# tensorchord/VectorChord-bm25

Hardware: AMD Instinct MI355X
Metric: queries/sec top-10 BM25, 10M synthetic docs; achieved HBM GB/s vs peak (higher is better)
Workload: dtype f64

## Files before the change

vectorchord-bm25_amd/csrc/scan_win.h:

```cpp
#ifndef VBM25_SCAN_WIN_H
#define VBM25_SCAN_WIN_H

#include "device_types.h"
#include "decode.h"
#include "topk_lds.h"
#include "block_fetch.h"
#include "topk_reg.h"

namespace vbm25 {

#pragma clang diagnostic push
#pragma clang diagnostic ignored "-Winline-asm"
constexpr int WN_T = 8;
#ifndef VBM25_WIN_WAVES_MAX
#define VBM25_WIN_WAVES_MAX 12
#endif
constexpr int wn_wave_lds(int mt) { return 8192 + 512 * mt + 256; }
constexpr int WN_WG_LDS = 2048 + 16;
constexpr int wn_waves(int mt, int rk) {
    const int by_lds = (163840 - WN_WG_LDS) / wn_wave_lds(mt);
    const int by_regs = rk <= 2 && mt <= 3 ? 16 : 12;
    const int n = by_lds < by_regs ? by_lds : by_regs;
    return n < VBM25_WIN_WAVES_MAX ? n : VBM25_WIN_WAVES_MAX;
}
constexpr bool wn_lane_addr(int mt, int rk) { return !(rk == 4 && mt >= 7); }
constexpr int WN_BM_WORDS = 2048;
constexpr int WN_SLOT = 256;
constexpr int WN_LIST = 64;
constexpr uint32_t WN_GRID = 256;

typedef __attribute__((address_space(3))) uint32_t wn_lds_u32;
struct WnBm {
    uint32_t base, mask;
};
__device__ __forceinline__ uint32_t wn_or_rtn(const WnBm bm, const uint32_t x, const uint32_t bit) {
    return __hip_atomic_fetch_or((wn_lds_u32 *)(((x >> 3) & bm.mask) | bm.base), bit, __ATOMIC_RELAXED, __HIP_MEMORY_SCOPE_WORKGROUP);
}
__device__ __forceinline__ void wn_or(const WnBm bm, const uint32_t x, const uint32_t bit) {
    (void)__hip_atomic_fetch_or((wn_lds_u32 *)(((x >> 3) & bm.mask) | bm.base), bit, __ATOMIC_RELAXED, __HIP_MEMORY_SCOPE_WORKGROUP);
}
template <int MT>
struct WinWave {
    alignas(16) uint16_t stage[MT * WN_SLOT];
    uint32_t list[WN_LIST];
};

__device__ __forceinline__ uint32_t wn_mbcnt(unsigned long long mask) {
    return __builtin_amdgcn_mbcnt_hi((uint32_t)(mask >> 32), __builtin_amdgcn_mbcnt_lo((uint32_t)mask, 0u));
}

template <bool RET, int MT>
__device__ __forceinline__ void wn_pair(WinWave<MT> &S, const WnBm bmbase, const uint2 v, const uint32_t r0, const uint32_t n,
                                        const uint32_t t, uint32_t &nd) {
    const uint32_t x0 = v.x & 0xffffu, x1 = v.x >> 16, x2 = v.y & 0xffffu, x3 = v.y >> 16;
    const uint32_t b0 = r0 < n ? 1u << (x0 & 31u) : 0u;
    const uint32_t b1 = r0 + 1u < n ? 1u << (x1 & 31u) : 0u;
    const uint32_t b2 = r0 + 2u < n ? 1u << (x2 & 31u) : 0u;
    const uint32_t b3 = r0 + 3u < n ? 1u << (x3 & 31u) : 0u;
    if (!RET) {
        wn_or(bmbase, x0, b0);
        wn_or(bmbase, x1, b1);
        wn_or(bmbase, x2, b2);
        wn_or(bmbase, x3, b3);
        return;
    }
    const uint32_t h0 = wn_or_rtn(bmbase, x0, b0) & b0;
    const uint32_t h1 = wn_or_rtn(bmbase, x1, b1) & b1;
    const uint32_t h2 = wn_or_rtn(bmbase, x2, b2) & b2;
    const uint32_t h3 = wn_or_rtn(bmbase, x3, b3) & b3;
    if (__ballot((h0 | h1 | h2 | h3) != 0u)) {
        uint32_t hm = (h0 ? 1u : 0u) | (h1 ? 2u : 0u) | (h2 ? 4u : 0u) | (h3 ? 8u : 0u);
        do {
            const bool has = hm != 0u;
            const uint32_t j = (uint32_t)__ffs((int)hm) - 1u;
            hm &= hm - 1u;
            const uint32_t x = j == 0u ? x0 : j == 1u ? x1 : j == 2u ? x2 : x3;
            const unsigned long long mk = __ballot(has);
            const uint32_t pos = nd + wn_mbcnt(mk);
            if (has && pos < (uint32_t)WN_LIST) S.list[pos] = x | t << 16 | 0x80000000u;
            nd += (uint32_t)__popcll(mk);
        } while (__ballot(hm != 0u));
    }
}

__device__ __forceinline__ void wn_load_run(unsigned long long &dst, const uint32_t voff, const unsigned long long sbase) {
    asm volatile("s_nop 4\n\tglobal_load_dwordx2 %0, %1, %2" : "=v"(dst) : "v"(voff), "s"(sbase));
}
__device__ __forceinline__ void wn_load_run_at(unsigned long long &dst, const unsigned long long vaddr) {
    asm volatile("global_load_dwordx2 %0, %1, off" : "=v"(dst) : "v"(vaddr));
}
__device__ __forceinline__ void wn_load_word(uint32_t &dst, const uint32_t *addr) {
    asm volatile("global_load_dword %0, %1, off" : "=v"(dst) : "v"(addr));
}
__device__ __forceinline__ void wn_load_theta(unsigned long long &dst, const uint32_t vzero, const unsigned long long *sbase) {
    asm volatile("s_nop 4\n\tglobal_load_dwordx2 %0, %1, %2 sc1" : "=v"(dst) : "v"(vzero), "s"(sbase));
}
#define WN_STR2(x) #x
#define WN_STR(x) WN_STR2(x)
#define WN_OPS1(b) "+v"(b[0])
#define WN_OPS2(b) WN_OPS1(b), "+v"(b[1])
#define WN_OPS3(b) WN_OPS2(b), "+v"(b[2])
#define WN_OPS4(b) WN_OPS3(b), "+v"(b[3])
#define WN_OPS5(b) WN_OPS4(b), "+v"(b[4])
#define WN_OPS6(b) WN_OPS5(b), "+v"(b[5])
#define WN_OPS7(b) WN_OPS6(b), "+v"(b[6])
#define WN_OPS8(b) WN_OPS7(b), "+v"(b[7])
template <int MT>
__device__ __forceinline__ void wn_wait_runs(unsigned long long (&b)[MT]) {
    static_assert(MT >= 1 && MT <= 8, "operand lists");
    if constexpr (MT == 1) asm volatile("s_waitcnt vmcnt(4)" : WN_OPS1(b));
    if constexpr (MT == 2) asm volatile("s_waitcnt vmcnt(5)" : WN_OPS2(b));
    if constexpr (MT == 3) asm volatile("s_waitcnt vmcnt(6)" : WN_OPS3(b));
    if constexpr (MT == 4) asm volatile("s_waitcnt vmcnt(7)" : WN_OPS4(b));
    if constexpr (MT == 5) asm volatile("s_waitcnt vmcnt(8)" : WN_OPS5(b));
    if constexpr (MT == 6) asm volatile("s_waitcnt vmcnt(9)" : WN_OPS6(b));
    if constexpr (MT == 7) asm volatile("s_waitcnt vmcnt(10)" : WN_OPS7(b));
    if constexpr (MT == 8) asm volatile("s_waitcnt vmcnt(11)" : WN_OPS8(b));
}
template <int MT>
__device__ __forceinline__ void wn_wait_words(uint32_t &ga, uint32_t &gb) {
    if constexpr (MT == 1) asm volatile("s_waitcnt vmcnt(1)" : "+v"(ga), "+v"(gb));
    if constexpr (MT == 2) asm volatile("s_waitcnt vmcnt(2)" : "+v"(ga), "+v"(gb));
    if constexpr (MT == 3) asm volatile("s_waitcnt vmcnt(3)" : "+v"(ga), "+v"(gb));
    if constexpr (MT == 4) asm volatile("s_waitcnt vmcnt(4)" : "+v"(ga), "+v"(gb));
    if constexpr (MT == 5) asm volatile("s_waitcnt vmcnt(5)" : "+v"(ga), "+v"(gb));
    if constexpr (MT == 6) asm volatile("s_waitcnt vmcnt(6)" : "+v"(ga), "+v"(gb));
    if constexpr (MT == 7) asm volatile("s_waitcnt vmcnt(7)" : "+v"(ga), "+v"(gb));
    if constexpr (MT == 8) asm volatile("s_waitcnt vmcnt(8)" : "+v"(ga), "+v"(gb));
}
template <int MT>
__device__ __forceinline__ void wn_wait_theta(unsigned long long &p) {
    if constexpr (MT == 1) asm volatile("s_waitcnt vmcnt(3)" : "+v"(p));
    if constexpr (MT == 2) asm volatile("s_waitcnt vmcnt(4)" : "+v"(p));
    if constexpr (MT == 3) asm volatile("s_waitcnt vmcnt(5)" : "+v"(p));
    if constexpr (MT == 4) asm volatile("s_waitcnt vmcnt(6)" : "+v"(p));
    if constexpr (MT == 5) asm volatile("s_waitcnt vmcnt(7)" : "+v"(p));
    if constexpr (MT == 6) asm volatile("s_waitcnt vmcnt(8)" : "+v"(p));
    if constexpr (MT == 7) asm volatile("s_waitcnt vmcnt(9)" : "+v"(p));
    if constexpr (MT == 8) asm volatile("s_waitcnt vmcnt(10)" : "+v"(p));
}
__device__ __forceinline__ void wn_wait_all(uint32_t &g) { asm volatile("s_waitcnt vmcnt(0)" : "+v"(g)); }
__device__ __forceinline__ unsigned long long wn_load_run_now(const uint16_t *addr) {
    unsigned long long v;
    asm volatile("global_load_dwordx2 %0, %1, off\n\ts_waitcnt vmcnt(0)" : "=v"(v) : "v"(addr));
    return v;
}
__device__ __forceinline__ uint32_t wn_load_u16_now(const uint16_t *addr) {
    uint32_t v;
    asm volatile("global_load_ushort %0, %1, off\n\ts_waitcnt vmcnt(0)" : "=v"(v) : "v"(addr));
    return v;
}
template <int MT>
__device__ __forceinline__ void wn_drain(unsigned long long (&a)[MT], unsigned long long (&b)[MT], uint32_t &g, uint32_t &g2, unsigned long long &p) {
    if constexpr (MT == 1) asm volatile("s_waitcnt vmcnt(0)" : WN_OPS1(a), WN_OPS1(b), "+v"(g), "+v"(g2), "+v"(p));
    if constexpr (MT == 2) asm volatile("s_waitcnt vmcnt(0)" : WN_OPS2(a), WN_OPS2(b), "+v"(g), "+v"(g2), "+v"(p));
    if constexpr (MT == 3) asm volatile("s_waitcnt vmcnt(0)" : WN_OPS3(a), WN_OPS3(b), "+v"(g), "+v"(g2), "+v"(p));
    if constexpr (MT == 4) asm volatile("s_waitcnt vmcnt(0)" : WN_OPS4(a), WN_OPS4(b), "+v"(g), "+v"(g2), "+v"(p));
    if constexpr (MT == 5) asm volatile("s_waitcnt vmcnt(0)" : WN_OPS5(a), WN_OPS5(b), "+v"(g), "+v"(g2), "+v"(p));
    if constexpr (MT == 6) asm volatile("s_waitcnt vmcnt(0)" : WN_OPS6(a), WN_OPS6(b), "+v"(g), "+v"(g2), "+v"(p));
    if constexpr (MT == 7) asm volatile("s_waitcnt vmcnt(0)" : WN_OPS7(a), WN_OPS7(b), "+v"(g), "+v"(g2), "+v"(p));
    if constexpr (MT == 8) asm volatile("s_waitcnt vmcnt(0)" : WN_OPS8(a), WN_OPS8(b), "+v"(g), "+v"(g2), "+v"(p));
}
__device__ __forceinline__ double wave_shl1_f64(double v) {
    const uint32_t lo = (uint32_t)__builtin_amdgcn_update_dpp(__double2loint(v), __double2loint(v), 0x130, 0xf, 0xf, false);
    const uint32_t hi = (uint32_t)__builtin_amdgcn_update_dpp(__double2hiint(v), __double2hiint(v), 0x130, 0xf, 0xf, false);
    return __hiloint2double((int)hi, (int)lo);
}
struct WnPend {
    bool valid, found, task;
    uint32_t x, p, w, gw;
    uint32_t cw;
};

constexpr uint32_t WN_LQ_SCORE = 1024;
constexpr uint32_t WN_LQ_DOC = 1536;
constexpr uint32_t WN_LQ_CNT = 1792;
constexpr uint32_t WN_LQ_G = 3, WN_LQ_WAVES = 12, WN_LQ_STRIDE = 4;
static_assert(WN_LQ_G * 256 <= WN_LQ_SCORE && WN_LQ_CNT + 4 <= 2048, "map, lists and counts share a filter");

template <int RK, bool LQ>
__device__ __forceinline__ void wn_merge_query(const DevIndex &ix, const uint32_t q, const uint32_t g, const uint32_t k, const uint32_t lane,
                                            uint32_t *map, double *sv_score, uint32_t *sv_doc, const uint32_t *lq) {
    const KernArgsP ca = cold_args();
    RegTopK<RK> rtop;
    rtop.init();
    const uint32_t L0 = q * g;
    constexpr uint32_t LQS = WN_LQ_STRIDE * (uint32_t)WN_BM_WORDS;
    unsigned long long theta = 0;
    if constexpr (LQ) {
        for (uint32_t i = 0; i < g; ++i) {
            const unsigned long long ti = (unsigned long long)lq[i * LQS + WN_LQ_CNT + 3u] << 32 | lq[i * LQS + WN_LQ_CNT + 2u];
            if (ti > theta) theta = ti;
        }
    } else {
        theta = __hip_atomic_load(&ca->bt.theta[q], __ATOMIC_RELAXED, __HIP_MEMORY_SCOPE_AGENT);
    }
    const uint32_t per_round = k <= 128u ? 16u : 2048u / k;
    uint32_t nsv = 0;
    bool ranked = true;
    for (uint32_t lb = 0; lb < g; lb += per_round) {
        uint32_t cnt = 0;
        if (lane < per_round && lb + lane < g) {
            if constexpr (LQ) cnt = min(lq[(lb + lane) * LQS + WN_LQ_CNT], k);
            else cnt = min(__hip_atomic_load(&ca->bt.res_cnt[L0 + lb + lane], __ATOMIC_RELAXED, __HIP_MEMORY_SCOPE_AGENT), k);
        }
        const uint32_t incl = wave_incl_scan_u32(cnt), excl = incl - cnt;
        const uint32_t total = (uint32_t)__builtin_amdgcn_readlane((int)incl, 63);
        for (uint32_t j = 0; j < cnt; ++j) map[excl + j] = lane << 16 | j;
        __builtin_amdgcn_wave_barrier();
        for (uint32_t e0 = 0; e0 < total; e0 += 64) {
            bool has = e0 + lane < total;
            double sc = 0;
            uint32_t d = 0;
            if (has) {
                const uint32_t ds = map[e0 + lane];
                if constexpr (LQ) {
                    const uint32_t *li = lq + (lb + (ds >> 16)) * LQS;
                    sc = reinterpret_cast<const double *>(li + WN_LQ_SCORE)[ds & 0xffffu];
                    d = li[WN_LQ_DOC + (ds & 0xffffu)];
                } else {
                    const size_t at = (size_t)(L0 + lb + (ds >> 16)) * k + (ds & 0xffffu);
                    sc = __longlong_as_double((long long)__hip_atomic_load(reinterpret_cast<unsigned long long *>(&ca->bt.res_score[at]), __ATOMIC_RELAXED,
                                                                           __HIP_MEMORY_SCOPE_AGENT));
                    d = __hip_atomic_load(&ca->bt.res_doc[at], __ATOMIC_RELAXED, __HIP_MEMORY_SCOPE_AGENT);
                }
                has = (unsigned long long)__double_as_longlong(sc) >= theta;
            }
            const unsigned long long hm = __ballot(has);
            if (ranked && nsv + (uint32_t)__popcll(hm) <= 64u) {
                if (has) {
                    const uint32_t at = nsv + wn_mbcnt(hm);
                    sv_score[at] = sc;
                    sv_doc[at] = d;
                }
                nsv += (uint32_t)__popcll(hm);
                continue;
            }
            if (ranked) {
                ranked = false;
                __builtin_amdgcn_wave_barrier();
                const bool hb = lane < nsv;
                rtop.offer(hb, hb ? sv_score[lane] : 0.0, hb ? sv_doc[lane] : 0u, k, lane);
            }
            rtop.offer(has, sc, d, k, lane);
        }
        __builtin_amdgcn_wave_barrier();
    }
    auto emit = [&](uint32_t i, double sc, uint32_t d) {
        const uint16_t *pl = ix.doc_payload + 3ull * d;
        unsigned long long *out = reinterpret_cast<unsigned long long *>(ca->bt.hits + (size_t)q * k + i);
        out[0] = (unsigned long long)__double_as_longlong(sc);
        out[1] = (unsigned long long)d | (unsigned long long)pl[0] << 32 | (unsigned long long)pl[1] << 48;
        out[2] = (unsigned long long)pl[2];
    };
    uint32_t n;
    if (ranked) {
        __builtin_amdgcn_wave_barrier();
        const bool mine = lane < nsv;
        const double sc = mine ? sv_score[lane] : 0.0;
        const uint32_t d = mine ? sv_doc[lane] : 0u;
        uint32_t place = 0;
        for (uint32_t j = 0; j < nsv; ++j) {
            const double sj = readlane_f64(sc, j);
            const uint32_t dj = (uint32_t)__builtin_amdgcn_readlane((int)d, (int)j);
            place += better(sj, dj, sc, d) ? 1u : 0u;
        }
        n = min(nsv, k);
        if (mine && place < k) emit(place, sc, d);
    } else {
        n = rtop.cnt;
#pragma unroll
        for (int r = 0; r < RK; ++r)
            if (r * 64 + lane < n) emit(r * 64 + lane, rtop.score[r], rtop.doc[r]);
    }
    uint32_t nf = 0;
    for (uint32_t i = lane; i < g; i += 64) {
        if constexpr (LQ) {
            nf += lq[i * LQS + WN_LQ_CNT + 1u] != 0u ? 1u : 0u;
        } else {
            nf += __hip_atomic_load(&ca->bt.item_failed[L0 + i], __ATOMIC_RELAXED, __HIP_MEMORY_SCOPE_AGENT) != 0u ? 1u : 0u;
            __hip_atomic_store(&ca->bt.item_failed[L0 + i], 0u, __ATOMIC_RELAXED, __HIP_MEMORY_SCOPE_AGENT);
            __hip_atomic_store(&ca->bt.res_cnt[L0 + i], 0u, __ATOMIC_RELAXED, __HIP_MEMORY_SCOPE_AGENT);
        }
    }
#pragma unroll
    for (int o = 32; o > 0; o >>= 1) nf += __shfl_xor(nf, o);
    if (lane == 0) {
        ca->bt.n_hits[q] = nf ? NONE32 : n;
        ca->bt.q_failed[q] = nf;
        ca->bt.theta_last[q] = theta;
        if constexpr (!LQ) {
            __hip_atomic_store(&ca->bt.theta[q], 0ull, __ATOMIC_RELAXED, __HIP_MEMORY_SCOPE_AGENT);
            __hip_atomic_store(&ca->bt.fused_state[1 + q], 0u, __ATOMIC_RELAXED, __HIP_MEMORY_SCOPE_AGENT);
        }
    }
}

template <int MT, int RK, bool FILT>
__global__ void __launch_bounds__(wn_waves(MT, RK) * 64, (wn_waves(MT, RK) + 3) / 4) scan_win_kernel(DevIndex ix, DevBatch bt) {
    constexpr int WN_WAVES = wn_waves(MT, RK), WN_WG = WN_WAVES * 64;
    static_assert(sizeof(WinWave<MT>) + WN_BM_WORDS * 4 == wn_wave_lds(MT), "wn_waves() knows the size");
    __shared__ alignas(8192) uint32_t BM[WN_WAVES * WN_BM_WORDS];
    __shared__ WinWave<MT> SW[WN_WAVES];
    __shared__ double S1[256];
    __shared__ uint32_t MQ[4];
    static_assert(sizeof(S1) + sizeof(MQ) == WN_WG_LDS, "wn_waves() knows the size");
    const uint32_t lane = threadIdx.x & 63;
    WinWave<MT> &S = SW[uni(threadIdx.x >> 6)];
    uint32_t *const bm = &BM[uni(threadIdx.x >> 6) * WN_BM_WORDS];
    WnBm bmbase;
    bmbase.base = uni((uint32_t)(uintptr_t)(wn_lds_u32 *)bm);
    bmbase.mask = 0x1ffcu;
    asm volatile("" : "+v"(bmbase.mask));
    const uint32_t k = bt.k, g = bt.win_g, n_items = bt.nq * g, NWIN = ix.n_win;
#ifdef VBM25_DEV
    const uint32_t dbg = bt.win_dbg;
#else
    constexpr uint32_t dbg = 0;
#endif
    const uint16_t *ids16 = reinterpret_cast<const uint16_t *>(ix.post_id16);
    auto item_of = [&](uint32_t item) -> uint32_t {
        const KernArgsP ca = cold_args();
        const uint32_t oo = ca->bt.order_on;
        if (oo == 1u) item = uni(ca->bt.item_order[item]);
        else if (oo == 2u) {
            const uint32_t full12 = (ca->bt.nq >> 2) * 12u;
            if (item < full12) {
                const uint32_t wgi = item / 12u, r = item - wgi * 12u;
                item = (wgi * 4u + (r & 3u)) * 3u + (r >> 2);
            }
        }
        return item;
    };
    auto query_terms = [&](const uint32_t q, uint32_t &tt, uint32_t &ti) {
        const KernArgsP ca = cold_args();
        const uint32_t qs = ca->bt.q_stride;
        const uint32_t qb = qs ? qs * q : uni(ca->bt.q_off[q]), qe = qs ? qs * (q + 1u) : uni(ca->bt.q_off[q + 1]);
        const uint32_t *idfb = ca->bt.id16_fb;
        tt = lane < qe - qb ? ca->bt.term_ids[qb + lane] : NONE32;
        ti = idfb && lane < qe - qb ? idfb[qb + lane] : NONE32;
    };
    const uint32_t n_waves = gridDim.x * (uint32_t)WN_WAVES;
    uint32_t drawn = blockIdx.x * (uint32_t)WN_WAVES + uni(threadIdx.x >> 6);
    bool pre = !(dbg & 8u) && drawn < n_items;
    uint32_t pre_item = 0, pre_tt = NONE32, pre_ti = NONE32;
    if (pre) {
        pre_item = item_of(drawn);
        query_terms(pre_item / g, pre_tt, pre_ti);
    }
    for (uint32_t i = threadIdx.x; i < 256u; i += WN_WG) S1[i] = ix.s1[i];
    if (threadIdx.x < 4u) MQ[threadIdx.x] = 0u;
#pragma unroll
    for (int i = 0; i < WN_BM_WORDS / 4 / 64; ++i) reinterpret_cast<uint4 *>(bm)[lane + 64 * i] = make_uint4(0, 0, 0, 0);
    __syncthreads();
#ifdef VBM25_PROFILE
    unsigned long long prof[16] = {0, 0, 0, 0, 0, 0, 0, 0, 0, 0, 0, 0, 0, 0, 0, 0};
    const unsigned long long prof_t0 = __builtin_readcyclecounter();
#endif

    uint32_t merge_q = NONE32;
    bool merge_lq = false;
    if (dbg & 8u) {
        uint32_t d0 = 0;
        if (lane == 0) d0 = atomicAdd(cold_args()->bt.work_ctr, 1u);
        drawn = uni(d0);
    }
    for (;;) {
        if (drawn >= n_items) break;
        const uint32_t item = pre ? pre_item : item_of(drawn);
        uint32_t w_lo, w_hi;
        PROF_T(t_item);
        const uint32_t q = item / g, part = item - q * g;
        {
            const KernArgsP ca = cold_args();
            if (g <= 16u && ca->bt.win_cut[g] != 0u) {
                w_lo = ca->bt.win_cut[part];
                w_hi = ca->bt.win_cut[part + 1u];
            } else {
                w_lo = (uint32_t)((unsigned long long)NWIN * part / g);
                w_hi = (uint32_t)((unsigned long long)NWIN * (part + 1u) / g);
            }
        }

        uint32_t m = 0, term = NONE32;
        uint32_t fbi = NONE32;
        {
            uint32_t tt = pre_tt, ti = pre_ti;
            if (!pre) query_terms(q, tt, ti);
            pre = false;
            const bool ok = tt < ix.n_terms;
            const unsigned long long okm = __ballot(ok);
            if (ok) {
                S.list[wn_mbcnt(okm)] = tt;
                if (wn_mbcnt(okm) < 32u) S.list[32u + wn_mbcnt(okm)] = ti;
            }
            m = (uint32_t)__popcll(okm);
            __builtin_amdgcn_wave_barrier();
            if (lane < min(m, (uint32_t)MT)) {
                term = S.list[lane];
                fbi = S.list[32u + lane];
            }
            __builtin_amdgcn_wave_barrier();
        }
        const bool act = lane < min(m, (uint32_t)MT);
        uint32_t fb = 0, wb = 0;
        double s0 = 0.0, kth = 0.0;
        {
            const KernArgsP ca = cold_args();
            const double *kub = ca->ix.term_kth_ub;
            if constexpr (FILT)
                if (query_filter(q)) kub = nullptr;
            if (act) {
                fb = ca->ix.term_first_block[term];
                if (fbi == NONE32) fbi = fb;
                s0 = ca->ix.term_s0[term];
                wb = ca->ix.term_win[term];
                if (kub) {
                    uint32_t kidx = 0;
                    while ((1u << kidx) < k) ++kidx;
                    kth = kub[(size_t)term * 9 + kidx];
                }
            }
        }
#ifndef VBM25_EXPERIMENT_WILD_NULL_TERMS
        if (!act) fbi = 0u;
#endif
        bool failed = m > (uint32_t)MT || __ballot(act && wb == NONE32) != 0ull;
        if (failed) m = 0;
        constexpr uint32_t mm = (uint32_t)MT;
        const uint32_t wbs = act && !failed ? wb : 0u;
        const unsigned long long pbase = (unsigned long long)ids16 + (act && !failed ? 256ull * fbi : 0ull);
        const uint32_t nw = w_hi - w_lo;
        failed = failed || nw > 63u;
        uint32_t wo[MT];
#pragma unroll
        for (int t = 0; t < MT; ++t)
            wo[t] = ix.win_off[(uint32_t)__builtin_amdgcn_readlane((int)wbs, t) + min(w_lo + lane, NWIN)];
        uint32_t wS = 0, wE = 0;
#pragma unroll
        for (int t = 0; t < MT; ++t) {
            if (lane == (uint32_t)t) {
                wS = (uint32_t)__builtin_amdgcn_readlane((int)wo[t], 0);
                wE = (uint32_t)__builtin_amdgcn_readlane((int)wo[t], (int)min(nw, 63u));
            }
        }
        uint32_t wA = 0, wB = wS;
#pragma unroll
        for (int o = 32; o > 0; o >>= 1) kth = fmax(kth, __shfl_xor(kth, o));
        unsigned long long th = (unsigned long long)__double_as_longlong(kth);
        {
            unsigned long long pg = __hip_atomic_load(&bt.theta[q], __ATOMIC_RELAXED, __HIP_MEMORY_SCOPE_AGENT);
            pg = ((unsigned long long)uni((uint32_t)(pg >> 32)) << 32) | uni((uint32_t)pg);
            if (lane == 0 && th > pg) atomicMax(&bt.theta[q], th);
            if (pg > th) th = pg;
        }
        if (lane == 0) {
            const KernArgsP ca = cold_args();
            Item rec;
            rec.q = q;
            rec.doc_lo = w_lo << 16;
            rec.doc_hi = (uint32_t)min((unsigned long long)w_hi << 16, (unsigned long long)ix.n_docs);
            rec.m = m;
            ca->bt.items[item] = rec;
            if (item == 0) *ca->bt.n_items = n_items;
            if (part == 0) ca->bt.q_item_base[q] = item;
            if (item + 1 == n_items) ca->bt.q_item_base[q + 1] = n_items;
        }

        RegTopK<RK> rtop;
        rtop.init();
        unsigned long long published = 0;
        auto offer = [&](bool has, double sc, uint32_t d) {
            has = has && (unsigned long long)__double_as_longlong(sc) >= th && (rtop.cnt < k || better(sc, d, rtop.kth_s, rtop.kth_d));
            if (!__ballot(has)) return;
            if constexpr (FILT) {
                if (const unsigned long long *fw = query_filter(q)) {
                    has = has && filter_keeps(fw, d);
                    if (!__ballot(has)) return;
                }
            }
            rtop.offer(has, sc, d, k, lane);
            if (rtop.cnt >= k) {
                const unsigned long long kb = (unsigned long long)__double_as_longlong(rtop.kth_s);
                if (kb > th) th = kb;
            }
        };

        const uint32_t lane8 = 8u * lane, lane4 = 4u * lane;
        unsigned long long vbase[wn_lane_addr(MT, RK) ? MT : 1];
        if constexpr (wn_lane_addr(MT, RK)) {
#pragma unroll
            for (int t = 0; t < MT; ++t) {
                vbase[t] = (((unsigned long long)(uint32_t)__builtin_amdgcn_readlane((int)(uint32_t)(pbase >> 32), t) << 32) |
                            (uint32_t)__builtin_amdgcn_readlane((int)(uint32_t)pbase, t)) + lane8;
                asm volatile("" : "+v"(vbase[t]));
            }
        }
        auto load_runs = [&](unsigned long long (&dst)[MT], const uint32_t i) {
            const uint32_t ic = min(i, 63u);
#pragma unroll
            for (int t = 0; t < MT; ++t) {
                const uint32_t o_al = (uint32_t)__builtin_amdgcn_readlane((int)wo[t], (int)ic) & ~3u;
                if constexpr (wn_lane_addr(MT, RK)) {
                    wn_load_run_at(dst[t], vbase[t] + 2ull * o_al);
                } else {
                    const unsigned long long a = (((unsigned long long)(uint32_t)__builtin_amdgcn_readlane((int)(uint32_t)(pbase >> 32), t) << 32) |
                                                  (uint32_t)__builtin_amdgcn_readlane((int)(uint32_t)pbase, t)) + 2ull * o_al;
                    wn_load_run(dst[t], lane8, a);
                }
            }
        };
        WnPend pa{}, pb{};
        unsigned long long pgv = 0;
        uint32_t vzero = 0;
        asm volatile("" : "+v"(vzero));
        unsigned long long bufa[MT], bufb[MT];
#pragma unroll
        for (int t = 0; t < MT; ++t) bufa[t] = bufb[t] = 0;
        load_runs(bufa, 0u);
        wn_load_theta(pgv, vzero, &bt.theta[q]);
        wn_load_word(pa.gw, ix.post_tfn);
        wn_load_word(pb.gw, ix.post_tfn);
        load_runs(bufb, 1u);
        wn_drain<MT>(bufa, bufb, pa.gw, pb.gw, pgv);

        const uint32_t inv_m = mm ? (65536u + mm - 1u) / mm : 0u, epp = mm ? 64u / mm : 0u;
        const uint32_t el = (lane * inv_m) >> 16, tl = mm ? lane - el * mm : 0u;
        const uint32_t fbl = (uint32_t)__shfl((int)fb, (int)tl);
        const uint32_t fbil = (uint32_t)__shfl((int)fbi, (int)tl);
        const double s0l = __shfl(s0, (int)tl);
        wB = (uint32_t)__shfl((int)wS, (int)tl);
        bool notf = false;
        struct C1S {
            bool task, found, more;
            uint32_t x, base, plo, len, slen;
        };
        auto c1_search = [&](const uint32_t e0, const uint32_t nd, auto &&hook) -> C1S {
            C1S r;
            const bool task = el < epp && e0 + el < nd;
            const uint32_t ent = S.list[task ? e0 + el : 0u];
            const uint32_t esl = ent & 31u;
            const uint32_t xs = S.stage[(task && !(ent >> 31) ? ((esl >> 2) + 5u * ((ent >> 11) & 1u)) * (uint32_t)WN_SLOT + ((ent >> 5) & 63u) * 4u + (esl & 3u) : 0u)];
            const uint32_t x = (ent >> 31) ? ent & 0xffffu : xs;
            const uint32_t plo = wA, phi = wB;
            const uint32_t pal = plo & ~3u, len = phi - plo;
            const uint16_t *sb = &S.stage[tl * WN_SLOT + (plo - pal)];
            uint32_t base = 0;
            const uint32_t slen = min(len, (uint32_t)WN_SLOT - (plo - pal));
            uint32_t n2 = task ? slen : 0u;
#define WN_BISECT_STEP(IT)                                              \
    {                                                                   \
        const uint32_t half = n2 >> 1;                                  \
        const uint32_t probe = sb[base + half];                         \
        hook(std::integral_constant<int, IT>());                        \
        if (probe <= x) base += half;                                   \
        n2 -= half;                                                     \
    }
            WN_BISECT_STEP(0) WN_BISECT_STEP(1) WN_BISECT_STEP(2) WN_BISECT_STEP(3) WN_BISECT_STEP(4) WN_BISECT_STEP(5) WN_BISECT_STEP(6) WN_BISECT_STEP(7)
#undef WN_BISECT_STEP
            uint32_t v_at = sb[base], v_last = sb[slen ? slen - 1u : 0u];
            asm volatile("" : "+v"(v_at), "+v"(v_last));
            r.found = task && len != 0u && v_at == x;
            r.more = task && !r.found && slen < len && v_last < x;
            r.task = task;
            r.x = x;
            r.base = base;
            r.plo = plo;
            r.len = len;
            r.slen = slen;
            return r;
        };
        auto c1_finish = [&](WnPend &d, const C1S &r, const uint32_t w) {
            bool found = r.found;
            uint32_t base = r.base;
            bool more = r.more;
            const uint32_t x = r.x;
            if (__ballot(more)) {
                const uint16_t *gb = ids16 + 128ull * fbil + r.plo;
                uint32_t lo = r.slen, hi = r.len;
                while (__ballot(more && lo < hi)) {
                    const uint32_t mid = (lo + hi) >> 1;
                    const uint32_t v = wn_load_u16_now(gb + (more ? mid : 0u));
                    if (more && lo < hi) {
                        if (v < x) lo = mid + 1u;
                        else hi = mid;
                    }
                }
                more = more && lo < r.len;
                const uint32_t v = wn_load_u16_now(gb + (more ? lo : 0u));
                if (more && v == x) {
                    found = true;
                    base = lo;
                }
            }
            uint32_t cw = 0;
            if (r.task && tl == 0u) {
                const uint32_t bit = 1u << (x & 31u);
                cw = __hip_atomic_fetch_and((wn_lds_u32 *)(((x >> 3) & bmbase.mask) | bmbase.base), ~bit, __ATOMIC_RELAXED, __HIP_MEMORY_SCOPE_WORKGROUP);
            }
            d.task = r.task;
            d.found = found;
            d.cw = cw;
            d.x = x;
            d.p = r.plo + base;
            d.w = w;
        };
        auto c1 = [&](WnPend &d, const uint32_t e0, const uint32_t nd, const uint32_t w) {
            const C1S r = c1_search(e0, nd, [](auto) {});
            c1_finish(d, r, w);
        };
        auto c1_request = [&](WnPend &d) { wn_load_word(d.gw, ix.post_tfn + (d.found ? 64ull * fbl + (d.p >> 1) : 0ull)); };
        struct C2R {
            bool okd;
            double acc;
            uint32_t doc;
        };
        auto c2_calc = [&](const WnPend &d) -> C2R {
            double c;
            {
                const uint32_t ww = d.gw >> ((d.p & 1u) * 8u);
                const uint32_t tfv = d.found ? ww & 0xffu : 0u, fn = tfv ? (ww >> 16) & 0xffu : 1u;
                notf = notf || (d.found && tfv == 0u);
                const double tf = (double)tfv;
                c = (tf * s0l) / (tf + S1[fn]);
            }
            const unsigned long long fm = __ballot(d.found);
            C2R r;
            r.okd = false;
            r.acc = 0.0;
            r.doc = d.w << 16 | d.x;
            {
                double sh = c;
                r.acc = c;
#pragma unroll
                for (int t = 1; t < MT; ++t) {
                    sh = wave_shl1_f64(sh);
                    r.acc += sh;
                }
            }
            if (d.task && tl == 0u) {
                const uint32_t my = (uint32_t)(fm >> lane) & ((1u << mm) - 1u);
                r.okd = ((d.cw >> (d.x & 31u)) & 1u) != 0u && (my & (my - 1u)) != 0u;
            }
            return r;
        };
        auto c2 = [&](const WnPend &d) {
            const C2R r = c2_calc(d);
            offer(r.okd, r.acc, r.doc);
        };
        struct C2Div {
            double num, den, sc0, rcp, f0, f1, f2, sc1, f3, mul, f4, q;
            bool vcc;
        };
        auto c2_div_begin = [&](const WnPend &d, C2Div &D) {
            const uint32_t ww = d.gw >> ((d.p & 1u) * 8u);
            const uint32_t tfv = d.found ? ww & 0xffu : 0u, fn = tfv ? (ww >> 16) & 0xffu : 1u;
            notf = notf || (d.found && tfv == 0u);
            const double tf = (double)tfv;
            D.num = tf * s0l;
            D.den = tf + S1[fn];
        };
        auto c2_div_step = [&](C2Div &D, auto itc) {
            constexpr int it = decltype(itc)::value;
            if constexpr (it == 0) {
                bool unused;
                D.sc0 = __builtin_amdgcn_div_scale(D.num, D.den, false, &unused);
                D.rcp = __builtin_amdgcn_rcp(D.sc0);
            }
            if constexpr (it == 1) D.f0 = __builtin_fma(-D.sc0, D.rcp, 1.0);
            if constexpr (it == 2) D.f1 = __builtin_fma(D.rcp, D.f0, D.rcp);
            if constexpr (it == 3) D.f2 = __builtin_fma(-D.sc0, D.f1, 1.0);
            if constexpr (it == 4) {
                D.sc1 = __builtin_amdgcn_div_scale(D.num, D.den, true, &D.vcc);
                D.f3 = __builtin_fma(D.f1, D.f2, D.f1);
            }
            if constexpr (it == 5) D.mul = D.sc1 * D.f3;
            if constexpr (it == 6) D.f4 = __builtin_fma(-D.sc0, D.mul, D.sc1);
            if constexpr (it == 7) D.q = __builtin_amdgcn_div_fixup(__builtin_amdgcn_div_fmas(D.f4, D.f3, D.mul, D.vcc), D.den, D.num);
        };
        auto c2_sum = [&](const WnPend &d, const double c) -> C2R {
            const unsigned long long fm = __ballot(d.found);
            C2R r;
            r.okd = false;
            r.doc = d.w << 16 | d.x;
            double sh = c;
            r.acc = c;
#pragma unroll
            for (int t = 1; t < MT; ++t) {
                sh = wave_shl1_f64(sh);
                r.acc += sh;
            }
            if (d.task && tl == 0u) {
                const uint32_t my = (uint32_t)(fm >> lane) & ((1u << mm) - 1u);
                r.okd = ((d.cw >> (d.x & 31u)) & 1u) != 0u && (my & (my - 1u)) != 0u;
            }
            return r;
        };

        auto window = [&](unsigned long long (&cur)[MT], const uint32_t w) -> bool {
            uint32_t nd = 0;
            wA = wB;
            PROF_T(t_0);
            wn_wait_runs<MT>(cur);
            PROF_T(t_1);
            PROF_ADD(1, t_0, t_1);
#ifdef VBM25_PROFILE
            unsigned long long t_p1 = t_1;
#endif
#pragma unroll
            for (int gq = 0; gq < (MT > 5 ? 2 : 1); ++gq) {
                constexpr int GT = 5;
                uint32_t ho[GT][4];
                uint32_t en[GT];
#pragma unroll
                for (int u = 0; u < GT; ++u)
#pragma unroll
                    for (int j = 0; j < 4; ++j) asm volatile("; ho undefined" : "=v"(ho[u][j]));
                if (!(dbg & 128u)) {
#pragma unroll
                    for (int u = 0; u < GT; ++u) {
                        const int t = GT * gq + u;
                        en[u] = 0;
                        if (t < MT) {
                            const uint32_t o_lo = (uint32_t)__builtin_amdgcn_readlane((int)wo[t < MT ? t : 0], (int)(w - w_lo));
                            const uint32_t o_hi = (uint32_t)__builtin_amdgcn_readlane((int)wo[t < MT ? t : 0], (int)(w - w_lo + 1u));
                            const uint32_t o_al = o_lo & ~3u;
                            en[u] = o_hi - o_al;
                            wB = tl == (uint32_t)t ? o_hi : wB;
                            const uint2 run = make_uint2((uint32_t)cur[t < MT ? t : 0], (uint32_t)(cur[t < MT ? t : 0] >> 32));
                            *reinterpret_cast<uint2 *>(&S.stage[t * WN_SLOT + 4u * lane]) = run;
                            if (lane4 < en[u] && !(dbg & 32u)) {
                                const uint32_t x0 = run.x & 0xffffu, x1 = run.x >> 16, x2 = run.y & 0xffffu, x3 = run.y >> 16;
                                if (t == 0) {
                                    wn_or(bmbase, x0, 1u << (x0 & 31u));
                                    wn_or(bmbase, x1, 1u << (x1 & 31u));
                                    wn_or(bmbase, x2, 1u << (x2 & 31u));
                                    wn_or(bmbase, x3, 1u << (x3 & 31u));
                                } else if (t == MT - 1) {
                                    ho[u][0] = *(wn_lds_u32 *)(((x0 >> 3) & bmbase.mask) | bmbase.base);
                                    ho[u][1] = *(wn_lds_u32 *)(((x1 >> 3) & bmbase.mask) | bmbase.base);
                                    ho[u][2] = *(wn_lds_u32 *)(((x2 >> 3) & bmbase.mask) | bmbase.base);
                                    ho[u][3] = *(wn_lds_u32 *)(((x3 >> 3) & bmbase.mask) | bmbase.base);
                                } else {
                                    ho[u][0] = wn_or_rtn(bmbase, x0, 1u << (x0 & 31u));
                                    ho[u][1] = wn_or_rtn(bmbase, x1, 1u << (x1 & 31u));
                                    ho[u][2] = wn_or_rtn(bmbase, x2, 1u << (x2 & 31u));
                                    ho[u][3] = wn_or_rtn(bmbase, x3, 1u << (x3 & 31u));
                                }
                            }
                            if (en[u] > (uint32_t)WN_SLOT) {
                                const uint16_t *rest = ids16 + 128ull * (uint32_t)__builtin_amdgcn_readlane((int)fbi, t) + 4u * lane;
                                const uint32_t n = o_hi - o_lo;
#pragma nounroll
                                for (uint32_t o = o_al + (uint32_t)WN_SLOT; o < o_hi; o += (uint32_t)WN_SLOT) {
                                    const unsigned long long mv = wn_load_run_now(rest + o);
                                    const uint2 more = make_uint2((uint32_t)mv, (uint32_t)(mv >> 32));
                                    if (t == 0) wn_pair<false, MT>(S, bmbase, more, o + 4u * lane - o_lo, n, (uint32_t)t, nd);
                                    else wn_pair<true, MT>(S, bmbase, more, o + 4u * lane - o_lo, n, (uint32_t)t, nd);
                                }
                            }
                        }
                    }
                }
#ifdef VBM25_PROFILE
                if (gq == 0) {
                    const unsigned long long t_2 = __builtin_readcyclecounter();
                    prof[2] += t_2 - t_1;
                    t_p1 = t_2;
                }
#endif
                if (!(dbg & (128u | 32u))) {
                    uint32_t flags = 0;
#pragma unroll
                    for (int u = 0; u < GT; ++u) {
                        const int t = GT * gq + u;
                        if (t >= 1 && t < MT) {
                            if (lane4 < en[u]) {
                                const uint32_t v0 = (uint32_t)cur[t < MT ? t : 0], v1 = (uint32_t)(cur[t < MT ? t : 0] >> 32);
                                uint32_t f = (ho[u][0] >> (v0 & 31u)) << 31;
                                f = __builtin_amdgcn_alignbit(ho[u][1] >> ((v0 >> 16) & 31u), f, 1);
                                f = __builtin_amdgcn_alignbit(ho[u][2] >> (v1 & 31u), f, 1);
                                f = __builtin_amdgcn_alignbit(ho[u][3] >> ((v1 >> 16) & 31u), f, 1);
                                flags |= (f >> 28) << (4 * u);
                            }
                        }
                    }
                    while (__ballot(flags != 0u)) {
                        const bool has = flags != 0u;
                        const uint32_t sl = (uint32_t)__ffs((int)flags) - 1u;
                        flags &= flags - 1u;
                        const unsigned long long mk = __ballot(has);
                        const uint32_t pos = nd + wn_mbcnt(mk);
                        if (has && pos < (uint32_t)WN_LIST) S.list[pos] = sl | lane << 5 | (uint32_t)gq << 11;
                        nd += (uint32_t)__popcll(mk);
                    }
                }
            }
            __builtin_amdgcn_wave_barrier();
            PROF_T(t_4);
#ifdef VBM25_PROFILE
            prof[3] += t_4 - t_p1;
#endif
            if (nd > (uint32_t)WN_LIST) failed = true;
#ifdef VBM25_PROFILE
            prof[0] += 1;
            prof[10] += nd;
#endif
            if (dbg & 4u) nd = 0;

            PROF_T(t_w0);
            PROF_ADD(4, t_4, t_w0);
            wn_wait_words<MT>(pa.gw, pb.gw);
            PROF_T(t_w1);
            PROF_ADD(5, t_w0, t_w1);
#ifdef VBM25_PROFILE
            unsigned long long t_w2 = 0;
#endif
            {
                const uint32_t nd1 = !failed && !(dbg & 2u) ? nd : 0u;
                C2Div dv;
                c2_div_begin(pa, dv);
                const C1S sa = c1_search(0u, nd1, [&](auto itc) { c2_div_step(dv, itc); });
                const C2R ra = c2_sum(pa, dv.q);
                offer(ra.okd, ra.acc, ra.doc);
                if (pb.valid) c2(pb);
                pb.valid = false;
                pa.found = pb.found = false;
                PROF_MARK(t_w2);
                PROF_ADD(6, t_w1, t_w2);
                c1_finish(pa, sa, w);
                pa.valid = nd1 != 0u;
                if (nd1 > epp) {
                    for (uint32_t e0 = ((nd1 - 1u) / epp) * epp; e0 >= 2u * epp; e0 -= epp) {
                        c1(pb, e0, nd1, w);
                        c1_request(pb);
                        wn_wait_all(pb.gw);
                        c2(pb);
                    }
                    pb.found = false;
                    c1(pb, epp, nd1, w);
                    pb.valid = true;
                }
            }
#ifdef VBM25_WIN_WIPE_STORES
            if (!(dbg & 64u))
#pragma unroll
                for (int i = 0; i < WN_BM_WORDS / 4 / 64; ++i) reinterpret_cast<uint4 *>(bm)[lane + 64 * i] = make_uint4(0, 0, 0, 0);
#else
            if (!(dbg & 64u)) {
#define WN_WIPE4(o) "ds_write_addtid_b32 %1 offset:" #o "\n\tds_write_addtid_b32 %1 offset:" #o "+256\n\tds_write_addtid_b32 %1 offset:" #o "+512\n\tds_write_addtid_b32 %1 offset:" #o "+768\n\t"
#define WN_WIPE32(o) WN_WIPE4(o) WN_WIPE4(o + 1024) WN_WIPE4(o + 2048) WN_WIPE4(o + 3072) WN_WIPE4(o + 4096) WN_WIPE4(o + 5120) WN_WIPE4(o + 6144) WN_WIPE4(o + 7168)
                asm volatile("s_mov_b32 m0, %0\n\ts_nop 0\n\t" WN_WIPE32(0) : : "s"(bmbase.base), "v"(vzero) : "m0", "memory");
#undef WN_WIPE32
#undef WN_WIPE4
            }
#endif
            PROF_T(t_5);
            PROF_ADD(7, t_w2, t_5);
            {
                wn_wait_theta<MT>(pgv);
                const unsigned long long pg = ((unsigned long long)uni((uint32_t)(pgv >> 32)) << 32) | uni((uint32_t)pgv);
                if (pg > th) th = pg;
            }
            wn_load_theta(pgv, vzero, &bt.theta[q]);
            c1_request(pa);
            c1_request(pb);
            load_runs(cur, w - w_lo + 2u);
            PROF_T(t_6);
            PROF_ADD(11, t_5, t_6);
            if (failed) return false;
            return true;
        };
        PROF_T(t_loop);
        for (uint32_t w = w_lo; w < w_hi; w += 2u) {
            if (!window(bufa, w)) break;
            if (w + 1u < w_hi && !window(bufb, w + 1u)) break;
        }
        PROF_T(t_loop_end);
        double cold_ub[MT];
#pragma unroll
        for (int t = 0; t < MT; ++t) {
            const uint32_t pS = (uint32_t)__builtin_amdgcn_readlane((int)wS, t), pE = (uint32_t)__builtin_amdgcn_readlane((int)wE, t);
            const uint32_t fbt = (uint32_t)__builtin_amdgcn_readlane((int)fb, t);
            const bool in = (uint32_t)t < mm && pE != pS && (pS >> 7) + lane <= ((pE - 1u) >> 7);
            cold_ub[t] = in ? ix.blk_ub[fbt + (pS >> 7) + lane] : 0.0;
        }
        wn_drain<MT>(bufa, bufb, pa.gw, pb.gw, pgv);
        uint32_t next_draw = n_items;
        if (lane == 0 && n_items > n_waves) next_draw = atomicAdd(cold_args()->bt.work_ctr, 1u);
        if (pa.valid && !failed) c2(pa);
        if (pb.valid && !failed) c2(pb);
        failed = failed || __ballot(notf) != 0ull;

        if (!failed && !(dbg & 1u)) {
            uint32_t hm0l = 0, hm0h = 0;
#pragma unroll
            for (int t = 0; t < MT; ++t) {
                const uint32_t pS = (uint32_t)__builtin_amdgcn_readlane((int)wS, t), pE = (uint32_t)__builtin_amdgcn_readlane((int)wE, t);
                const uint32_t fbt = (uint32_t)__builtin_amdgcn_readlane((int)fb, t);
                const bool in = (uint32_t)t < mm && pE != pS && (pS >> 7) + lane <= ((pE - 1u) >> 7);
                const double ub = cold_ub[t];
                const unsigned long long hm = __ballot(in && (unsigned long long)__double_as_longlong(ub) >= th);
                if (lane == (uint32_t)t) {
                    hm0l = (uint32_t)hm;
                    hm0h = (uint32_t)(hm >> 32);
                }
            }
            for (uint32_t t = 0; t < mm; ++t) {
                const uint32_t pS = (uint32_t)__builtin_amdgcn_readlane((int)wS, (int)t), pE = (uint32_t)__builtin_amdgcn_readlane((int)wE, (int)t);
                if (pE == pS) continue;
                const uint32_t fbt = (uint32_t)__builtin_amdgcn_readlane((int)fb, (int)t);
                const double s0t = readlane_f64(s0, t);
                const uint32_t bS = pS >> 7, bE = (pE - 1u) >> 7;
                for (uint32_t b0 = bS; b0 <= bE; b0 += 64u) {
                    unsigned long long hm = (unsigned long long)(uint32_t)__builtin_amdgcn_readlane((int)hm0h, (int)t) << 32 |
                                            (uint32_t)__builtin_amdgcn_readlane((int)hm0l, (int)t);
                    if (b0 != bS) {
                        const bool in = b0 + lane <= bE;
                        double ub = 0.0;
                        if (in) ub = ix.blk_ub[fbt + b0 + lane];
                        hm = __ballot(in && (unsigned long long)__double_as_longlong(ub) >= th);
                    }
                    for (; hm != 0ull; hm &= hm - 1ull) {
                        const uint32_t blk = fbt + b0 + (uint32_t)__ffsll((long long)hm) - 1u;
                        const unsigned long long ubb = (unsigned long long)__double_as_longlong(ix.blk_ub[blk]);
                        if ((((unsigned long long)uni((uint32_t)(ubb >> 32)) << 32) | uni((uint32_t)ubb)) < th) continue;
                        const uint4 bm = uni4(ix.blk_meta[blk]);
                        const uint32_t n = bm.w & 0xff, md = (bm.w >> 8) & 0xff, mt = (bm.w >> 16) & 0xff;
                        const uint8_t *body = ix.blob + 8ull * bm.z;
                        uint32_t dd0, dd1, tt0, tt1;
                        decode_doc_ids(body, md, n, bm.x, lane, dd0, dd1);
                        decode_fields(body + ((payload_bytes(md, n) + 7u) & ~7u), mt, n, lane, tt0, tt1);
                        const uchar2 fnn = reinterpret_cast<const uchar2 *>(ix.post_fn + 128ull * blk)[lane];
#pragma nounroll
                        for (uint32_t j = 0; j < 2u; ++j) {
                            const uint32_t d = j ? dd1 : dd0, wd = d >> 16;
                            const double tf = (double)(2u * lane + j < n ? (j ? tt1 : tt0) : 1u);
                            const double sc = (tf * s0t) / (tf + S1[j ? fnn.y : fnn.x]);
                            bool cand = 2u * lane + j < n && wd >= w_lo && wd < w_hi && (unsigned long long)__double_as_longlong(sc) >= th &&
                                        (rtop.cnt < k || better(sc, d, rtop.kth_s, rtop.kth_d));
                            if (!__ballot(cand)) continue;
                            for (uint32_t t2 = 0; t2 < mm; ++t2) {
                                if (t2 == t) continue;
                                const uint32_t wb2 = (uint32_t)__builtin_amdgcn_readlane((int)wbs, (int)t2);
                                const uint16_t *run = ids16 + 128ull * (uint32_t)__builtin_amdgcn_readlane((int)fbi, (int)t2);
                                uint32_t lo = 0, hi = 0;
                                if (cand) {
                                    lo = ix.win_off[wb2 + wd];
                                    hi = ix.win_off[wb2 + wd + 1u];
                                }
                                while (__ballot(lo < hi)) {
                                    const uint32_t mid = (lo + hi) >> 1;
                                    if (lo < hi) {
                                        if ((uint32_t)run[mid] < (d & 0xffffu)) lo = mid + 1u;
                                        else hi = mid;
                                    }
                                }
                                if (cand && lo < ix.win_off[wb2 + wd + 1u] && (uint32_t)run[lo] == (d & 0xffffu)) cand = false;
                            }
                            offer(cand, sc, d);
                        }
                    }
                }
            }
        }
        bool lq = false;
        if constexpr (WN_WAVES == (int)WN_LQ_WAVES) {
            const KernArgsP ca = cold_args();
            lq = ca->bt.win_fuse != 0u && ca->bt.order_on == 2u && g == WN_LQ_G && n_items <= n_waves && !(dbg & 8u) &&
                 blockIdx.x * (uint32_t)WN_WAVES + uni(threadIdx.x >> 6) < (ca->bt.nq >> 2) * WN_LQ_WAVES;
        }
        if (rtop.cnt >= k && !lq) {
            const unsigned long long kb = (unsigned long long)__double_as_longlong(rtop.kth_s);
            if (kb > published && lane == 0) atomicMax(&bt.theta[q], kb);
        }

#ifdef VBM25_PROFILE
        {
            const unsigned long long t_end = __builtin_readcyclecounter();
            prof[12] += 1;
            prof[9] += t_loop_end - t_loop;
            prof[8] += t_loop - t_item;
            prof[13] += t_end - t_loop_end;
        }
#endif
        const uint32_t nres = failed ? 0u : rtop.cnt;
        const KernArgsP ce = cold_args();
        if (lq) {
            double *const ls = reinterpret_cast<double *>(bm + WN_LQ_SCORE);
#pragma unroll
            for (int r = 0; r < RK; ++r)
                if (r * 64 + lane < nres) {
                    ls[r * 64 + lane] = rtop.score[r];
                    bm[WN_LQ_DOC + r * 64 + lane] = rtop.doc[r];
                }
            if (lane == 0) {
                bm[WN_LQ_CNT] = nres;
                bm[WN_LQ_CNT + 1u] = failed ? 1u : 0u;
                bm[WN_LQ_CNT + 2u] = (uint32_t)th;
                bm[WN_LQ_CNT + 3u] = (uint32_t)(th >> 32);
                if (failed) *ce->bt.fail_any = 1u;
            }
            uint32_t *const mq = &MQ[uni(threadIdx.x >> 6) & 3u];
            asm volatile("s_waitcnt lgkmcnt(0)" ::: "memory");
            uint32_t done = 0;
            if (lane == 0) done = __hip_atomic_fetch_add(mq, 1u, __ATOMIC_RELAXED, __HIP_MEMORY_SCOPE_WORKGROUP);
            asm volatile("" ::: "memory");
            if ((uni(done) & 0xffu) == g - 1u) {
                merge_q = q;
                merge_lq = true;
            } else {
                if (rtop.cnt >= k && lane == 0) atomicMax(&bt.theta[q], (unsigned long long)__double_as_longlong(rtop.kth_s));
                asm volatile("s_waitcnt vmcnt(0)" ::: "memory");
                done = 0;
                if (lane == 0) done = __hip_atomic_fetch_add(mq, 0x100u, __ATOMIC_RELAXED, __HIP_MEMORY_SCOPE_WORKGROUP);
                if (lane == 0 && (done >> 8) == g - 1u) __hip_atomic_store(&bt.theta[q], 0ull, __ATOMIC_RELAXED, __HIP_MEMORY_SCOPE_AGENT);
            }
        } else {
            const size_t list = (size_t)item * ce->bt.lpi;
#pragma unroll
            for (int r = 0; r < RK; ++r)
                if (r * 64 + lane < nres) {
                    __hip_atomic_store(reinterpret_cast<unsigned long long *>(&ce->bt.res_score[list * k + r * 64 + lane]),
                                       (unsigned long long)__double_as_longlong(rtop.score[r]), __ATOMIC_RELAXED, __HIP_MEMORY_SCOPE_AGENT);
                    __hip_atomic_store(&ce->bt.res_doc[list * k + r * 64 + lane], rtop.doc[r], __ATOMIC_RELAXED, __HIP_MEMORY_SCOPE_AGENT);
                }
            if (lane == 0) {
                __hip_atomic_store(&ce->bt.res_cnt[list], nres, __ATOMIC_RELAXED, __HIP_MEMORY_SCOPE_AGENT);
                __hip_atomic_store(&ce->bt.item_failed[item], failed ? 0x101u : 0u, __ATOMIC_RELAXED, __HIP_MEMORY_SCOPE_AGENT);
                if (failed) *ce->bt.fail_any = 1u;
            }
            if (ce->bt.win_fuse) {
                asm volatile("s_waitcnt vmcnt(0)" ::: "memory");
                uint32_t done = 0;
                if (lane == 0) done = atomicAdd(&ce->bt.fused_state[1 + q], 1u);
                if (uni(done) == g - 1u) merge_q = q;
            }
        }
        drawn = ((dbg & 8u) ? 0u : n_waves) + uni(next_draw);
    }
    if (merge_q != NONE32) {
        PROF_T(t_m0);
        double *const sv_score = reinterpret_cast<double *>(&S.stage[0]);
        uint32_t *const sv_doc = reinterpret_cast<uint32_t *>(&S.stage[256]);
        if (merge_lq) {
            wn_merge_query<RK, true>(ix, merge_q, g, k, lane, bm, sv_score, sv_doc, &BM[(uni(threadIdx.x >> 6) & 3u) * WN_BM_WORDS]);
            uint32_t done = 0;
            if (lane == 0) done = __hip_atomic_fetch_add(&MQ[uni(threadIdx.x >> 6) & 3u], 0x100u, __ATOMIC_RELAXED, __HIP_MEMORY_SCOPE_WORKGROUP);
            if (lane == 0 && (done >> 8) == g - 1u) __hip_atomic_store(&bt.theta[merge_q], 0ull, __ATOMIC_RELAXED, __HIP_MEMORY_SCOPE_AGENT);
        } else wn_merge_query<RK, false>(ix, merge_q, g, k, lane, bm, sv_score, sv_doc, nullptr);
        PROF_T(t_m1);
        PROF_ADD(14, t_m0, t_m1);
    }
#ifdef VBM25_PROFILE
    if (bt.prof && lane == 0) {
        unsigned long long *o = bt.prof + ((size_t)blockIdx.x * WN_WAVES + (threadIdx.x >> 6)) * 16;
        for (int i = 0; i < 16; ++i) o[i] = prof[i];
        o[15] = __builtin_readcyclecounter() - prof_t0;
    }
#endif
}
#pragma clang diagnostic pop

}

#endif
```

Baseline: 6.137 million.

## Interleave two pending-entry bisect searches and sums in window scan

Adds a 'wide' path for configurations other than the largest RK=4 tile sizes. When more than one group of epp list entries is pending, the two groups (pa and pb) run their LDS bisection searches and division steps together in one pass, and their sums are offered back to back. The aim is to overlap two dependent LDS probe chains and hide latency that the serial per-group processing left exposed. The cost is higher register pressure, and the pending-state handoff between iterations changes.

```diff
diff --git a/vectorchord-bm25_amd/csrc/scan_win.h b/vectorchord-bm25_amd/csrc/scan_win.h
--- a/vectorchord-bm25_amd/csrc/scan_win.h
+++ b/vectorchord-bm25_amd/csrc/scan_win.h
@@ -24,6 +24,11 @@
     return n < VBM25_WIN_WAVES_MAX ? n : VBM25_WIN_WAVES_MAX;
 }
 constexpr bool wn_lane_addr(int mt, int rk) { return !(rk == 4 && mt >= 7); }
+#ifdef VBM25_WIN_NARROW
+constexpr bool wn_wide(int, int) { return false; }
+#else
+constexpr bool wn_wide(int mt, int rk) { return !(rk == 4 && mt >= 5); }
+#endif
 constexpr int WN_BM_WORDS = 2048;
 constexpr int WN_SLOT = 256;
 constexpr int WN_LIST = 64;
@@ -570,7 +575,48 @@
             r.slen = slen;
             return r;
         };
-        auto c1_finish = [&](WnPend &d, const C1S &r, const uint32_t w) {
+        auto c1_search2 = [&](const uint32_t nd, C1S &ra, C1S &rb, auto &&hook) {
+            const bool taska = el < epp && el < nd, taskb = el < epp && epp + el < nd;
+            const uint32_t enta = S.list[taska ? el : 0u], entb = S.list[taskb ? epp + el : 0u];
+            const uint32_t esla = enta & 31u, eslb = entb & 31u;
+            const uint32_t xsa = S.stage[(taska && !(enta >> 31) ? ((esla >> 2) + 5u * ((enta >> 11) & 1u)) * (uint32_t)WN_SLOT + ((enta >> 5) & 63u) * 4u + (esla & 3u) : 0u)];
+            const uint32_t xsb = S.stage[(taskb && !(entb >> 31) ? ((eslb >> 2) + 5u * ((entb >> 11) & 1u)) * (uint32_t)WN_SLOT + ((entb >> 5) & 63u) * 4u + (eslb & 3u) : 0u)];
+            const uint32_t xa = (enta >> 31) ? enta & 0xffffu : xsa, xb = (entb >> 31) ? entb & 0xffffu : xsb;
+            const uint32_t plo = wA, phi = wB;
+            const uint32_t pal = plo & ~3u, len = phi - plo;
+            const uint16_t *sb = &S.stage[tl * WN_SLOT + (plo - pal)];
+            uint32_t basea = 0, baseb = 0;
+            const uint32_t slen = min(len, (uint32_t)WN_SLOT - (plo - pal));
+            uint32_t n2 = taska ? slen : 0u;
+#define WN_BISECT_STEP2(IT)                                             \
+    {                                                                   \
+        const uint32_t half = n2 >> 1;                                  \
+        const uint32_t probea = sb[basea + half];                       \
+        const uint32_t probeb = sb[baseb + half];                       \
+        hook(std::integral_constant<int, IT>());                        \
+        if (probea <= xa) basea += half;                                \
+        if (probeb <= xb) baseb += half;                                \
+        n2 -= half;                                                     \
+    }
+            WN_BISECT_STEP2(0) WN_BISECT_STEP2(1) WN_BISECT_STEP2(2) WN_BISECT_STEP2(3) WN_BISECT_STEP2(4) WN_BISECT_STEP2(5) WN_BISECT_STEP2(6) WN_BISECT_STEP2(7)
+#undef WN_BISECT_STEP2
+            uint32_t va_at = sb[basea], vb_at = sb[baseb], v_last = sb[slen ? slen - 1u : 0u];
+            asm volatile("" : "+v"(va_at), "+v"(vb_at), "+v"(v_last));
+            ra.found = taska && len != 0u && va_at == xa;
+            rb.found = taskb && len != 0u && vb_at == xb;
+            ra.more = taska && !ra.found && slen < len && v_last < xa;
+            rb.more = taskb && !rb.found && slen < len && v_last < xb;
+            ra.task = taska;
+            rb.task = taskb;
+            ra.x = xa;
+            rb.x = xb;
+            ra.base = basea;
+            rb.base = baseb;
+            ra.plo = rb.plo = plo;
+            ra.len = rb.len = len;
+            ra.slen = rb.slen = slen;
+        };
+        auto c1_finish =[&](WnPend &d, const C1S &r, const uint32_t w) {
             bool found = r.found;
             uint32_t base = r.base;
             bool more = r.more;
@@ -816,8 +862,40 @@
 #ifdef VBM25_PROFILE
             unsigned long long t_w2 = 0;
 #endif
-            {
-                const uint32_t nd1 = !failed && !(dbg & 2u) ? nd : 0u;
+            uint32_t nd1 = !failed && !(dbg & 2u) ? nd : 0u;
+            if (dbg & 256u) nd1 = min(nd1, epp);
+            bool wide = false;
+            if constexpr (wn_wide(MT, RK)) wide = nd1 > epp;
+            if (wide) {
+                C2Div dva, dvb;
+                c2_div_begin(pa, dva);
+                c2_div_begin(pb, dvb);
+                C1S sa, sb;
+                c1_search2(nd1, sa, sb, [&](auto itc) {
+                    c2_div_step(dva, itc);
+                    c2_div_step(dvb, itc);
+                });
+                asm volatile("" : "+v"(dva.q), "+v"(dvb.q));
+                const C2R ra = c2_sum(pa, dva.q);
+                const C2R rb = c2_sum(pb, dvb.q);
+                offer(ra.okd, ra.acc, ra.doc);
+                offer(rb.okd, rb.acc, rb.doc);
+                PROF_MARK(t_w2);
+                PROF_ADD(6, t_w1, t_w2);
+                c1_finish(pa, sa, w);
+                c1_finish(pb, sb, w);
+                pa.valid = nd1 != 0u;
+                pb.valid = nd1 > epp;
+                if (nd1 > 2u * epp) {
+                    WnPend pc{};
+                    for (uint32_t e0 = ((nd1 - 1u) / epp) * epp; e0 >= 2u * epp; e0 -= epp) {
+                        c1(pc, e0, nd1, w);
+                        c1_request(pc);
+                        wn_wait_all(pc.gw);
+                        c2(pc);
+                    }
+                }
+            } else {
                 C2Div dv;
                 c2_div_begin(pa, dv);
                 const C1S sa = c1_search(0u, nd1, [&](auto itc) { c2_div_step(dv, itc); });
@@ -830,7 +908,7 @@
                 PROF_ADD(6, t_w1, t_w2);
                 c1_finish(pa, sa, w);
                 pa.valid = nd1 != 0u;
-                if (nd1 > epp) {
+                if (!wn_wide(MT, RK) && nd1 > epp) {
                     for (uint32_t e0 = ((nd1 - 1u) / epp) * epp; e0 >= 2u * epp; e0 -= epp) {
                         c1(pb, e0, nd1, w);
                         c1_request(pb);
```

After: 6.136 million (median of 4 runs). About the same (-0.0%).
